# MathThyMod/GP_emu_UQSA

Hardware: AMD Instinct MI355X
Metric: log-marginal-likelihood evals/sec at n=16384 d=10 fp64; 1/2/4/8 GPU (higher is better)
Workload: dtype f64

## Files before the change

### gp_emu_uqsa_amd/csrc/gpemu.hip

```cpp
#include <hip/hip_runtime.h>

#include <algorithm>
#include <array>
#include <atomic>
#include <map>
#include <cmath>
#include <cstdio>
#include <cstdlib>
#include <cstring>
#include <limits>
#include <string>
#include <vector>

#include "../../include/gpemu.h"
#include "gpemu_kernels.hpp"
#include "gpemu_small.hpp"
#include "gpemu_tiny.hpp"
#include "gpemu_snb.hpp"
#include "gpemu_ozaki.hpp"
#include "gpemu_pivchol.hpp"
#include "gpemu_postgrad.hpp"
#include "gpemu_host_alloc.hpp"

using namespace gpe;
// ... 112 lines not shown
  size_t xs_cap = 0, xsw_cap = 0;
  double* dsmall = nullptr;
  double* dtiny = nullptr;
  int tiny_ek = 0, tiny_eg = 0;
  bool tiny_dirty = true;
  double* dsnb = nullptr;
  long long snb_np = 0;
  int snb_hc = 0, snb_mf = 0;
  bool snb_dirty = true;
  double onel_tag = 0.0;
  int oz_on = 1, oz_nmod = OZ_MAXMOD;
  int oz_min_np = 6144;
  int oz_np2 = 0, oz_list_len = 0;
  long long oz_npad = 0;
  OzConst oz_c{};
  int8_t* dozp = nullptr;
  int8_t* dozr = nullptr;
  int* dozx = nullptr;
  unsigned* dozl = nullptr;
  double* dozt = nullptr;
  hipEvent_t ev_oz = nullptr;
  std::vector<OzTriPair> oz_tri;
  int oz_tri_min = 8192;
  double oz_lauum_ops = 0.0;
  int oz_chol = 1, oz_chol_min = OZ_CHOL_MIN;
  OzTriPair oz_chol_q{};
  long long oz_chol_loff = 0;
  int oz_chol_llen = 0;
  double oz_chol_ops = 0.0;
  bool oz_chol_ready = false;
  bool oz_l21_valid = false;
  std::vector<hipEvent_t> oev;
  size_t oev_used = 0;
  double oz_ms = 0.0, oz_launches = 0.0, oz_ops = 0.0, oz_flops64 = 0.0;
  int dbg_skip_wait = -1;
  size_t small_cap = 0;

  double* hpin = nullptr;
  size_t hpin_cap = 0;

  float* dX32 = nullptr;
  size_t x32_cap = 0;
  bool x32_valid = false;
  float* dK32 = nullptr;
  size_t k32_cap = 0;
  hipEvent_t ev_pipe[2] = {nullptr, nullptr};
// ... 145 lines not shown
    return fail(c, GPE_ERR_ARG, "internal error: bad correlation family");
  if (a.d > 32) {
    const dim3 g(nblocks), b(256);
    if (a.fam == FAM_MATERN32) hipLaunchKernelGGL(k_pairs_wide<FAM_MATERN32>, g, b, 0, c->stream, a);
    else if (a.fam == FAM_MATERN52) hipLaunchKernelGGL(k_pairs_wide<FAM_MATERN52>, g, b, 0, c->stream, a);
    else hipLaunchKernelGGL(k_pairs_wide<FAM_GAUSS>, g, b, 0, c->stream, a);
    HIPCHK(c, hipGetLastError());
    return GPE_OK;
  }
  static constexpr int widths[] = {2, 4, 6, 8, 10, 12, 16, 20, 24, 32};
  int dm = 32;
  for (int w : widths)
    if (a.d <= w) { dm = w; break; }
  PairArgs a2 = a;
  while (a2.csplit < 4 && nblocks * a2.csplit * 2 <= 512) a2.csplit *= 2;
  const dim3 g(nblocks * a2.csplit), b(256);
  if (a.fam == FAM_MATERN32) launch_pairs_fam<FAM_MATERN32>(dm, g, b, c->stream, a2);
  else if (a.fam == FAM_MATERN52) launch_pairs_fam<FAM_MATERN52>(dm, g, b, c->stream, a2);
  else launch_pairs_fam<FAM_GAUSS>(dm, g, b, c->stream, a2);
  HIPCHK(c, hipGetLastError());
  return GPE_OK;
}

template <int FAM>
static void launch_contract(gpe_ctx* c, int d, int P, dim3 gc, int nblk, const double* rdiag, int cs) {
  const long long np = c->n_pad;
  const int bucket = std::max(d, P);
  if (d > 32 || P > 33) {
    hipLaunchKernelGGL(k_contract_wide<FAM>, dim3(nblk), dim3(256), 0, c->stream, c->tr.A, np, c->dXw, d, c->dWa, np, P, (int)c->n, c->dcpart, c->dinfo, 0, 0ll, rdiag);
  } else if (d == 10 && P <= 13) {
    hipLaunchKernelGGL((k_contract<10, 13, FAM>), gc, dim3(256), 0, c->stream, c->tr.A, np, c->dXw, d, c->dWa, np, P, (int)c->n, c->dcpart, c->dinfo, 0, 0ll, rdiag, cs);
  } else if (bucket <= 8) {
    hipLaunchKernelGGL((k_contract<8, 9, FAM>), gc, dim3(256), 0, c->stream, c->tr.A, np, c->dXw, d, c->dWa, np, P, (int)c->n, c->dcpart, c->dinfo, 0, 0ll, rdiag, cs);
  } else if (bucket <= 16) {
    hipLaunchKernelGGL((k_contract<16, 17, FAM>), gc, dim3(256), 0, c->stream, c->tr.A, np, c->dXw, d, c->dWa, np, P, (int)c->n, c->dcpart, c->dinfo, 0, 0ll, rdiag, cs);
  } else {
    hipLaunchKernelGGL((k_contract<32, 33, FAM>), gc, dim3(256), 0, c->stream, c->tr.A, np, c->dXw, d, c->dWa, np, P, (int)c->n, c->dcpart, c->dinfo, 0, 0ll, rdiag, cs);
  }
}

int launch_gemm_range(gpe_ctx* c, const Launch& L, hipStream_t st = nullptr) {
  if (!st) st = c->stream;
  const size_t lds = G_LDS_LAUNCH_DOUBLES * sizeof(double);
  const GemmProb* pr = c->dprobs + L.first;
  const unsigned* tl = (L.list >= 0) ? c->dtiles + L.list : nullptr;
  if (c->prof) {
    if (c->gev_used + 2 > c->gev.size()) {
      for (int i = 0; i < 256; ++i) {
        hipEvent_t e;
        HIPCHK(c, hipEventCreate(&e));
        c->gev.push_back(e);
      }
    }
    HIPCHK(c, hipEventRecord(c->gev[c->gev_used], st));
  }
  const dim3 g(L.tiles), b(256);
  if (L.cdef) {
    switch (L.kind) {
      case 0: hipLaunchKernelGGL((k_gemm<false, false, false, true>), g, b, lds, st, pr, L.count, tl, c->dinfo, L.ticket); break;
      case 1: hipLaunchKernelGGL((k_gemm<true, false, false, true>), g, b, lds, st, pr, L.count, tl, c->dinfo, L.ticket); break;
// ... 1131 lines not shown
    c->oz_chol_q = q;
    c->oz_chol_loff = (long long)all.size();
    c->oz_chol_llen = (int)ls.size();
    all.insert(all.end(), ls.begin(), ls.end());
    c->oz_chol_ops = 2.0 * OZ_T * OZ_T * (double)q.Pa * N * (nts * (nts + 1) / 2);
    planes = std::max(planes, (size_t)N * q.Pb * q.Pa);
    resid = std::max(resid, (size_t)N * (nts * (size_t)(nts + 1) / 2) * OZ_T * OZ_T);
    nex = std::max(nex, (size_t)q.Pb);
    c->oz_chol_ready = true;
  }
  CHK(dalloc(c, &c->dozp, planes));
  CHK(dalloc(c, &c->dozr, resid));
  CHK(dalloc(c, &c->dozx, nex));
  CHK(dalloc(c, &c->dozt, scratch));
  CHK(dalloc(c, &c->dozl, all.size()));
  HIPCHK(c, hipMemcpy(c->dozl, all.data(), all.size() * sizeof(unsigned), hipMemcpyHostToDevice));
  c->oz_c = oz_consts(N, np2);
  c->oz_np2 = np2;
  c->oz_npad = c->n_pad;
  return GPE_OK;
}

int oz_gemm_crt(gpe_ctx* c, const OzGemm& g, const OzCrt& r, int nti, double ops, double flops64,
                hipStream_t st = nullptr) {
  if (!st) st = c->stream;
  const OzConst& k = c->oz_c;
  if (c->prof) {
    while (c->oev_used + 2 > c->oev.size()) {
      hipEvent_t e;
      HIPCHK(c, hipEventCreate(&e));
      c->oev.push_back(e);
    }
    HIPCHK(c, hipEventRecord(c->oev[c->oev_used], st));
  }
  hipLaunchKernelGGL(k_oz_gemm, dim3(k.nmod * g.list_len), dim3(256), OZ_LDS, st, g, k);
  if (c->prof) {
    HIPCHK(c, hipEventRecord(c->oev[c->oev_used + 1], st));
    c->oev_used += 2;
    c->oz_launches += 1.0;
    c->oz_ops += ops;
    c->oz_flops64 += flops64;
  }
  hipLaunchKernelGGL(k_oz_crt, dim3((g.tri ? nti * (nti + 1) / 2 : nti * g.ntj) * 16), dim3(256), 0, st, r, k);
  HIPCHK(c, hipGetLastError());
  return GPE_OK;
}

int chol_schur(gpe_ctx* c, Fact& F, hipStream_t st, bool with_aug) {
  const Plan& pl = F.plan;
  const OzTriPair& q = c->oz_chol_q;
  if (!c->oz_chol_ready || q.h != pl.split_h) return fail(c, GPE_ERR_STATE, "internal error: split Cholesky without an int8 plan");
  if (with_aug) CHK(launch_gemm_range(c, pl.launches[pl.aug_mid], st));
  const long long ld = F.n_pad;
  oz_l21_launch(st, c->oz_c, q, F.A + (long long)q.h * TILE, ld, c->dozp, c->dozx);
  HIPCHK(c, hipGetLastError());
  const int nts = q.Pb / OZ_T;
  const long long pA = (long long)q.Pb * q.Pa, rb = (long long)nts * (nts + 1) / 2 * OZ_T * OZ_T;
  OzGemm g;
  g.a = g.b = OzOpnd{c->dozp, pA, q.Pa, 0};
  g.list = c->dozl + c->oz_chol_loff;
  g.list_len = c->oz_chol_llen;
  g.K = q.Pa;
  g.kbeg = 0;
  g.kend = 0;
  g.tri = 1;
  g.ntj = 0;
  g.res = c->dozr;
  g.res_bytes = rb;
  OzCrt r{c->dozr, rb, 1, 0, c->dozx, c->dozx, F.A + (long long)q.h * TILE * (ld + 1), ld, q.Rb, q.Rb, 1, -1.0};
  r.acc = 1;
  CHK(oz_gemm_crt(c, g, r, nts, c->oz_chol_ops, (double)q.Rb * q.Rb * q.Ra, st));
  c->oz_l21_valid = true;
  return GPE_OK;
}

int lauum_ozaki(gpe_ctx* c, Fact& F) {
  CHK(oz_prepare(c, F));
  const int np = (int)F.n_pad, np2 = c->oz_np2, NT2 = np2 / OZ_T;
  const OzConst& k = c->oz_c;
  const long long pb = oz_plane_bytes(np2), rb = (long long)NT2 * (NT2 + 1) / 2 * OZ_T * OZ_T;
  c->oz_l21_valid = false;
  hipLaunchKernelGGL(k_oz_colexp, dim3((np2 + 3) / 4), dim3(256), 0, c->stream, F.B, (long long)F.n_pad, np, np2,
                     k.beta, c->dozx);
  hipLaunchKernelGGL(k_oz_split, dim3(np2, (np2 + 256 * OZ_SPLIT_ROWS - 1) / (256 * OZ_SPLIT_ROWS)), dim3(256), 0,
                     c->stream, F.B, (long long)F.n_pad, np, np2, c->dozx, c->dozp, pb, k);
  OzGemm g;
  g.a = g.b = OzOpnd{c->dozp, pb, 0, np2};
  g.list = c->dozl;
  g.list_len = c->oz_list_len;
  g.K = np2;
  g.kbeg = 1;
  g.kend = 0;
  g.tri = 1;
  g.ntj = 0;
  g.res = c->dozr;
  g.res_bytes = rb;
  OzCrt r{c->dozr, rb, 1, 0, c->dozx, c->dozx, F.A, (long long)F.n_pad, np, np, 1, 1.0};
  return oz_gemm_crt(c, g, r, NT2, c->oz_lauum_ops, (double)np * np * np / 3.0);
}

const OzTriPair* oz_pair(const gpe_ctx* c, int t0, int h, int t1) {
  for (const OzTriPair& q : c->oz_tri)
    if (q.t0 == t0 && q.h == h && q.t1 == t1) return &q;
  return nullptr;
}

int oz_l21(gpe_ctx* c, Fact& F, const OzTriPair& q, hipStream_t st) {
  c->oz_l21_valid = false;
  oz_l21_launch(st, c->oz_c, q, F.A + (long long)q.h * TILE + (long long)q.t0 * TILE * F.n_pad, F.n_pad, c->dozp, c->dozx);
  HIPCHK(c, hipGetLastError());
  return GPE_OK;
}

int oz_l21_ahead(gpe_ctx* c, Fact& F, int t0, int h, int t1) {
  CHK(oz_prepare(c, F));
  const OzTriPair* q = oz_pair(c, t0, h, t1);
  if (!q) return fail(c, GPE_ERR_STATE, "internal error: TRTRI pair without an int8 plan");
  if (!c->ev_oz) HIPCHK(c, hipEventCreateWithFlags(&c->ev_oz, hipEventDisableTiming));
  HIPCHK(c, hipEventRecord(c->ev_fork, c->stream));
  HIPCHK(c, hipStreamWaitEvent(c->stream2, c->ev_fork, 0));
  CHK(oz_l21(c, F, *q, c->stream2));
// ... 88 lines not shown
  gpe_ctx* c = new gpe_ctx();
  c->device = device;
  c->aux.desc_base = AUX_DESC_BASE;
  {
    const char* ea = std::getenv("GPEMU_AUG");
    c->tr.aug = !(ea && std::string(ea) == "0");
  }
  {
    const char* e2 = std::getenv("GPEMU_POTRF");
    if (e2) {
      const std::string m(e2);
      c->potrf_group = m == "group" || m == "auto";
      c->potrf_mode = m == "group" ? 1 : (m == "auto" ? 0 : 2);
    }
    if (const char* eg = std::getenv("GPEMU_GROUP_P0")) c->grp_p0 = std::max(1, std::atoi(eg));
    if (const char* eg = std::getenv("GPEMU_GROUP_STRIDE")) c->grp_stride = std::max(0, std::atoi(eg));
    if (const char* ep = std::getenv("GPEMU_CHOL_PRIO")) c->chol_prio = std::atoi(ep) != 0;
    if (const char* et = std::getenv("GPEMU_TINY")) c->tiny = std::atoi(et) != 0;
    if (const char* ed = std::getenv("GPEMU_DEBUG_SKIP_WAIT")) c->dbg_skip_wait = std::atoi(ed);
    if (const char* eo = std::getenv("GPEMU_OZAKI")) c->oz_on = std::atoi(eo) != 0;
    if (const char* en = std::getenv("GPEMU_OZAKI_MIN_NP")) c->oz_min_np = std::max(512, std::atoi(en));
    if (const char* em = std::getenv("GPEMU_OZAKI_MODULI")) c->oz_nmod = std::max(8, std::min(OZ_MAXMOD, std::atoi(em)));
    if (const char* et = std::getenv("GPEMU_OZAKI_TRI_MIN")) c->oz_tri_min = std::max(512, std::atoi(et));
    if (const char* ec = std::getenv("GPEMU_OZAKI_CHOL")) c->oz_chol = std::max(0, std::min(3, std::atoi(ec)));
    if (const char* ec = std::getenv("GPEMU_OZAKI_CHOL_MIN")) c->oz_chol_min = std::max(256, std::atoi(ec));
    if (const char* es = std::getenv("GPEMU_POTRF_SB")) {
      c->potrf_sb = std::max(1, std::min(8, std::atoi(es)));
      if (const char* colon = std::strchr(es, ':')) c->potrf_sb_min = std::max(0, std::atoi(colon + 1));
    }
    if (const char* e3 = std::getenv("GPEMU_POTRF_W")) {
      c->potrf_groups.clear();
      std::string spec(e3);
      size_t pos = 0;
      while (pos < spec.size()) {
        size_t end = spec.find(',', pos);
        if (end == std::string::npos) end = spec.size();
        const std::string item = spec.substr(pos, end - pos);
        const size_t colon = item.find(':');
        const int w = std::atoi(item.substr(0, colon).c_str());
        const int lim = colon == std::string::npos ? 0 : std::atoi(item.substr(colon + 1).c_str());
        if (w >= 1 && w <= 8) c->potrf_groups.push_back({w, lim});
        pos = end + 1;
      }
    }
  }
  if (hipSetDevice(device) != hipSuccess || hipStreamCreateWithFlags(&c->stream, hipStreamNonBlocking) != hipSuccess ||
// ... 431 lines not shown
    c->gev_used = 0;
    c->gemm_launches = c->gemm_flops = c->gemm_ms = 0.0;
    c->oev_used = 0;
    c->oz_ms = c->oz_launches = c->oz_ops = c->oz_flops64 = 0.0;
  }
  const bool one_launch = c->tiny && kernel_fam(kernel) == FAM_GAUSS;
  if (one_launch && c->NB == 1 && d <= TINY_DM && q + 1 <= TINY_DM)
    return tiny_objective(c, gp4ml, kernel, hp, n_hp, fitnug, nu, s2, rscale, want_grad != 0, llh_out, grad_out,
                          sigma2_out);
  if (one_launch && c->NB >= 2 && c->NB <= SNB_MAXNB && d <= TINY_DM && q + 1 <= TINY_DM)
    return snb_objective(c, gp4ml, kernel, hp, n_hp, fitnug, nu, s2, rscale, want_grad != 0, llh_out, grad_out,
                         sigma2_out);

  CHK(factor_and_invert(c, kernel, hp, nu, s2, rscale, want_grad != 0, true));
  const int P = q + 1;
  const long long np = c->n_pad;
  const int NBt = c->tr.NB;
  CHK(ensure_pinned(c, (size_t)P * P + NBt + 64));
  CHK(gram_async(c, c->dZ, np, P, (int)np));
  HIPCHK(c, hipMemcpyAsync(c->hpin + P * P, c->tr.logdet, NBt * sizeof(double), hipMemcpyDeviceToHost, c->stream));
  HIPCHK(c, hipMemcpyAsync(c->hpin + P * P + NBt, c->dinfo, sizeof(int), hipMemcpyDeviceToHost, c->stream));
  HIPCHK(c, hipEventRecord(c->ev_host, c->stream));
  ev_rec(c, 4);
  if (want_grad) CHK(oz_use(c) ? lauum_ozaki(c, c->tr) : lauum(c, c->tr));
  ev_rec(c, 5);
  HIPCHK(c, hipEventSynchronize(c->ev_host));
  std::vector<double> G(c->hpin, c->hpin + (size_t)P * P);
  int info = 0;
  std::memcpy(&info, c->hpin + P * P + NBt, sizeof(int));
  if (info == GEMM_WAIT_TIMEOUT) return fail(c, GPE_ERR_HIP, "internal error: Cholesky panel wait timed out");
  double logdetA = 0.0;
  for (int k = 0; k < NBt; ++k) logdetA += c->hpin[P * P + k];
  logdetA *= 2.0;
  if (info != 0) {
    c->err = "matrix not positive definite (pivot " + std::to_string(info) + ")";
    return GPE_NOT_PD;
  }
  SmallAlgebra sa = small_from_gram(G, P);
  if (!sa.ok) {
    c->err = "H^T A^-1 H not positive definite";
    return GPE_NOT_PD;
  }
  const double n = (double)c->n;
  double llh, sig2, cfac, gscale;
  if (gp4ml) {
    llh = 0.5 * (sa.quad + logdetA + sa.logdetQ + (n - q) * std::log(2.0 * M_PI));
    sig2 = s2;
// ... 7 lines not shown
  }
  *llh_out = llh;
  if (sigma2_out) *sigma2_out = sig2;
  if (!want_grad) {
    ev_rec(c, 6);
    ev_rec(c, 7);
    goto done;
  }
  {
    CHK(ensure_pinned(c, (size_t)P * P + 8));
    const std::vector<double> T2 = small_t2(sa, q, cfac);
    std::memcpy(c->hpin, T2.data(), T2.size() * sizeof(double));
    HIPCHK(c, hipMemcpyAsync(c->dT2, c->hpin, T2.size() * sizeof(double), hipMemcpyHostToDevice, c->stream));
    CHK(apply_small(c, c->dZ, np, P, c->dT2, P, c->dR2, np, (int)np, c->dinfo));
    CHK(skinny(c, true, c->tr.B, np, c->NB, c->NB, true, c->dR2, np, P, c->dWa, np));
    ev_rec(c, 6);
    const double* rdiag = (gp4ml && !kernel_alt(kernel) && c->has_r) ? c->dr : nullptr;
    const int nblk = c->NB * (c->NB + 1) / 2;
    int cs = 1;
    if (!(d > 32 || P > 33))
      while (cs < 4 && nblk * cs * 2 <= 512) cs *= 2;
    const dim3 gc(nblk * cs);
    const int fam = kernel_fam(kernel);
    if (fam == FAM_MATERN32) launch_contract<FAM_MATERN32>(c, d, P, gc, nblk, rdiag, cs);
    else if (fam == FAM_MATERN52) launch_contract<FAM_MATERN52>(c, d, P, gc, nblk, rdiag, cs);
    else launch_contract<FAM_GAUSS>(c, d, P, gc, nblk, rdiag, cs);
    HIPCHK(c, hipGetLastError());
    hipLaunchKernelGGL(k_reduce_rows, dim3(d + 3), dim3(256), 0, c->stream, c->dcpart, nblk * cs, d + 3, c->dcsum);
    HIPCHK(c, hipGetLastError());
    ev_rec(c, 7);
    HIPCHK(c, hipMemcpyAsync(c->hpin, c->dcsum, (d + 3) * sizeof(double), hipMemcpyDeviceToHost, c->stream));
    HIPCHK(c, hipStreamSynchronize(c->stream));
    const double* red = c->hpin;
    double coff, cdiag;
    kernel_consts(kernel, nu, true, &coff, &cdiag);
    small_grad(red, d, kernel_alt(kernel), nu, fitnug, gp4ml, gscale, s2, coff, cdiag, n_hp,
               grad_out, rdiag != nullptr);
  }
done:
  if (c->prof) {
    HIPCHK(c, hipStreamSynchronize(c->stream));
    float ms;
    const int pairs[7][2] = {{0, 1}, {1, 2}, {2, 3}, {4, 5}, {3, 4}, {5, 7}, {0, 7}};
    for (int i = 0; i < 7; ++i) {
      ms = 0.f;
      (void)hipEventElapsedTime(&ms, c->ev[pairs[i][0]], c->ev[pairs[i][1]]);
      c->phase_ms[i] = ms;
    }
    double g = 0.0;
// ... 80 lines not shown
    c->pl_len = (int)l.size();
    c->pl_nti = nti;
    c->pl_ntj = ntj;
  }
  CHK(grow_buf(c, &c->dpkp, &c->pkp_cap, (size_t)N * pB));
  CHK(grow_buf(c, &c->dpke, &c->pke_cap, (size_t)mp2));
  CHK(grow_buf(c, &c->dpres, &c->pres_cap, (size_t)N * rb));
  hipLaunchKernelGGL(k_oz_rowexp<false>, dim3(mp2 / 4), dim3(256), 0, st, Ks, (long long)np, (int)mp, mp2, np, 0, k.beta,
                     c->dpke);
  hipLaunchKernelGGL(k_oz_split_rect<false>, dim3(mp2, (np2 + 2047) / 2048), dim3(256), 0, st, Ks, (long long)np,
                     (int)mp, np, 0, c->dpke, c->dpkp, pB, (long long)np2, np2, k);
  OzGemm g;
  g.a = OzOpnd{c->dpxp, (long long)np2 * np2, np2, 0};
  g.b = OzOpnd{c->dpkp, pB, np2, 0};
  g.list = c->dpl;
  g.list_len = c->pl_len;
  g.K = np2;
  g.kbeg = 0;
  g.kend = 1;
  g.tri = 0;
  g.ntj = ntj;
  g.res = c->dpres;
  g.res_bytes = rb;
  hipLaunchKernelGGL(k_oz_gemm, dim3(N * g.list_len), dim3(256), OZ_LDS, st, g, k);
  OzCrt r{c->dpres, rb, 0, ntj, c->dpxe, c->dpke, V, (long long)np, np, (int)mp, 0, 1.0};
  hipLaunchKernelGGL(k_oz_crt, dim3((unsigned)(nti * ntj * 16)), dim3(256), 0, st, r, k);
  HIPCHK(c, hipGetLastError());
  return GPE_OK;
}

static int ensure_ainv(gpe_ctx* c) {
  if (c->ainv_valid) return GPE_OK;
  CHK(ensure_linv(c));
  CHK(lauum(c, c->tr));
  c->ainv_valid = true;
  return GPE_OK;
}

int gpe_solve(gpe_ctx* c, int32_t ncols, const double* B, double* X) {
  CHK(check_ready(c));
  if (!c->factor_valid) return fail(c, GPE_ERR_STATE, "no resident factor (call gpe_factor)");
  if (ncols <= 0 || !B || !X) return fail(c, GPE_ERR_ARG, "bad solve args");
  CHK(ensure_linv(c));
  const long long np = c->n_pad, n = c->n;
  for (int c0 = 0; c0 < ncols; c0 += SK_PMAX) {
    const int cc = std::min(SK_PMAX, ncols - c0);
// ... 1197 lines not shown
```

### gp_emu_uqsa_amd/csrc/gpemu_ozaki.hpp

```cpp
#pragma once
#include <algorithm>
#include <array>
#include <cmath>
#include <cstdlib>
#include <cstring>
#include <utility>
#include <vector>

namespace gpe {

constexpr int OZ_T = 256;
constexpr int OZ_SK = 64;
constexpr int OZ_NBUF = 4;
constexpr int OZ_OPND = OZ_T * OZ_SK;
constexpr int OZ_LDS = OZ_NBUF * 2 * OZ_OPND;
constexpr int OZ_MAXMOD = 16;
constexpr int OZ_MAX_K = (1 << 17) - 128;

struct OzConst {
  int m[OZ_MAXMOD];
  int c16[OZ_MAXMOD];
  float inv[OZ_MAXMOD];
  double rhi[OZ_MAXMOD];
  double rlo[OZ_MAXMOD];
  double Md;
  int nmod;
// ... 79 lines not shown
  long long ld;
  int np2;
};
__device__ __forceinline__ const int8_t* oz_tile_rows(const OzOpnd& o, int t, int k, long long& ld) {
  if (o.ld == 0) {
    ld = o.np2 - OZ_T * t;
    return o.p + oz_panel_off(t, o.np2) + (k - OZ_T * t);
  }
  ld = o.ld;
  return o.p + (long long)OZ_T * t * o.ld + k;
}

struct OzGemm {
  OzOpnd a, b;
  const unsigned* list;
  int list_len;
  int K, kbeg, kend;
  int tri, ntj;
  int8_t* res;
  long long res_bytes;
  int kdiv = 1;
  int ti0 = 0;
};
__device__ __forceinline__ long long oz_res_tile(int tri, int ntj, int ti, int tj) {
  return tri ? (long long)ti * (ti + 1) / 2 + tj : (long long)ti * ntj + tj;
}

static __global__ void __launch_bounds__(256, 1) k_oz_gemm(OzGemm g, OzConst cst) {
  extern __shared__ __attribute__((aligned(16))) double lds_d[];
  int8_t* lds = reinterpret_cast<int8_t*>(lds_d);
  const int l = (int)blockIdx.x / g.list_len;
  const unsigned ent = g.list[(int)blockIdx.x - l * g.list_len];
  if (ent == 0xffffffffu) return;
  const int ti = (int)(ent >> 16), tj = (int)(ent & 0xffffu);
  const int kb = g.kbeg == 1 ? OZ_T * ti : (g.kbeg == 2 ? OZ_T * tj : (g.kbeg == 3 ? 128 * ((2 * ti) / g.kdiv) : 0));
  const int ke = g.kend == 1 ? min(g.K, OZ_T * (ti + 1)) : g.K;
  const int tid = threadIdx.x, lane = tid & 63;
  const int wave = __builtin_amdgcn_readfirstlane(tid >> 6);
  const int wm = (wave >> 1) * 128, wn = (wave & 1) * 128;
  OzOpnd oa = g.a, ob = g.b;
  oa.p += (long long)l * oa.plane_bytes;
  ob.p += (long long)l * ob.plane_bytes;
  long long lda, ldb;
  const int kp = (lane & 3) ^ ((lane >> 4) & 3);
  const int8_t* sa = oz_tile_rows(oa, ti, kb, lda);
  const int8_t* sb = oz_tile_rows(ob, tj, kb, ldb);
  sa += (long long)(16 * wave + (lane >> 2)) * lda + 16 * kp;
  sb += (long long)(16 * wave + (lane >> 2)) * ldb + 16 * kp;
  auto stage = [&](int s) {
    int8_t* As = lds + (s & (OZ_NBUF - 1)) * 2 * OZ_OPND;
    int8_t* Bs = As + OZ_OPND;
#pragma unroll
    for (int p = 0; p < 4; ++p) {
      const int w = wave + 4 * p;
      oz_glds16(sa + (long long)p * 64 * lda + (long long)s * OZ_SK, As + 16 * w * OZ_SK);
      oz_glds16(sb + (long long)p * 64 * ldb + (long long)s * OZ_SK, Bs + 16 * w * OZ_SK);
    }
  };
  oz_v16i acc[4][4];
// ... 117 lines not shown
    const double rh = cst.rhi[l], rl = cst.rlo[l];
#pragma unroll
    for (int r = 0; r < 16; ++r) {
      const double cv = (double)(int)(int8_t)((unsigned)w[r >> 2] >> (8 * (r & 3)));
      shi[r] = fma(cv, rh, shi[r]);
      slo[r] = fma(cv, rl, slo[r]);
    }
  }
  const int em = g.exr[gm];
  const double sc = g.alpha * cst.Md;
#pragma unroll
  for (int r = 0; r < 16; ++r) {
    const int gn = gn0 + (r & 3) + 8 * (r >> 2);
    if (gn >= g.cols || (g.lower128 && (gm >> 7) < (gn >> 7))) continue;
    const double v = (shi[r] - rint(shi[r])) + slo[r];
    const int en = g.exc[gn];
    double* dst = g.C + (gm - OZ_T * g.ti0 + (long long)gn * g.ldc);
    const double s = ldexp(sc, -(em + en));
    if (em == OZ_EX_NAN || en == OZ_EX_NAN) *dst = __builtin_nan("");
    else *dst = g.acc ? fma(v, s, *dst) : v * s;
  }
}

__device__ __forceinline__ bool oz_keep(int mask, int r, int k) {
  return mask == 1 ? k >= r : (mask == 2 ? k <= r : true);
}

template <bool TRANS>
static __global__ void __launch_bounds__(256) k_oz_rowexp(const double* __restrict__ src, long long ld, int R, int Rp,
                                                          int Kv, int mask, int beta, int* __restrict__ ex) {
  if constexpr (!TRANS) {
    const int lane = threadIdx.x & 63, r = blockIdx.x * 4 + (threadIdx.x >> 6);
    if (r >= Rp) return;
    double mx = 0.0;
    if (r < R)
      for (int k = lane; k < Kv; k += 64)
        if (oz_keep(mask, r, k)) mx = oz_pmax(mx, fabs(src[k + (long long)r * ld]));
    for (int off = 32; off > 0; off >>= 1) mx = oz_pmax(mx, __shfl_xor(mx, off, 64));
    if (lane == 0) ex[r] = oz_ex_of(mx, beta);
  } else {
    __shared__ double red[4][64];
    const int rl = threadIdx.x & 63, q = threadIdx.x >> 6, r = blockIdx.x * 64 + rl;
    const int k0 = blockIdx.y * 256;
    double mx = 0.0;
    if (r < R)
#pragma unroll 8
      for (int u = 0; u < 64; ++u) {
        const int k = k0 + 4 * u + q;
        if (k < Kv && oz_keep(mask, r, k)) mx = oz_pmax(mx, fabs(src[r + (long long)k * ld]));
      }
    red[q][rl] = mx;
    __syncthreads();
    if (q == 0 && r < R) {
      mx = oz_pmax(oz_pmax(red[0][rl], red[1][rl]), oz_pmax(red[2][rl], red[3][rl]));
      if (!(mx <= 1.7976931348623157e308)) atomicMax(ex + r, OZ_IL_BAD);
      else if (mx > 0.0) atomicMax(ex + r, ilogb(mx) + 2048);
    }
  }
}
static __global__ void __launch_bounds__(256) k_oz_il_to_ex(int* __restrict__ ex, int Rp, int beta) {
  const int r = blockIdx.x * 256 + threadIdx.x;
  if (r < Rp) ex[r] = ex[r] >= OZ_IL_BAD ? OZ_EX_NAN : (ex[r] > 0 ? (beta - 1) - (ex[r] - 2048) : 0);
}

__device__ __forceinline__ unsigned oz_res8(double x, double m, double im, int mi) {
  const double q = rint(x * im);
  int r = (int)fma(-q, m, x);
  r = r > 127 ? r - mi : (r < -128 ? r + mi : r);
  return (unsigned)r & 0xffu;
}

template <bool TRANS>
static __global__ void __launch_bounds__(256) k_oz_split_rect(const double* __restrict__ src, long long ld, int R,
                                                              int Kv, int mask, const int* __restrict__ ex,
                                                              int8_t* __restrict__ planes, long long plane_bytes,
                                                              long long ldp, int Kp, OzConst cst) {
  if constexpr (!TRANS) {
    const int r = blockIdx.x;
    const int k0 = ((int)blockIdx.y * 256 + (int)threadIdx.x) * 8;
    if (k0 >= Kp) return;
    const int e = ex[r];
    double xs[8];
    const double* p = src + k0 + (long long)r * ld;
    const int side = mask == 1 ? (k0 >= r ? 1 : (k0 + 7 < r ? 0 : 2))
                   : (mask == 2 ? (k0 + 7 <= r ? 1 : (k0 > r ? 0 : 2)) : 1);
    if (r < R && k0 + 8 <= Kv && side == 1 && ((reinterpret_cast<uintptr_t>(p) & 15) == 0)) {
#pragma unroll
      for (int u = 0; u < 8; u += 2) {
        const double2 v = *reinterpret_cast<const double2*>(p + u);
        xs[u] = v.x;
        xs[u + 1] = v.y;
      }
    } else {
#pragma unroll
      for (int u = 0; u < 8; ++u) {
        const int k = k0 + u;
        xs[u] = (side != 0 && r < R && k < Kv && oz_keep(mask, r, k)) ? p[u] : 0.0;
      }
    }
#pragma unroll
    for (int u = 0; u < 8; ++u) xs[u] = e == OZ_EX_NAN ? 0.0 : rint(ldexp(xs[u], e));
    int8_t* dst = planes + (long long)r * ldp + k0;
    for (int l = 0; l < cst.nmod; ++l) {
      const double m = (double)cst.m[l], im = 1.0 / m;
      unsigned w0 = 0u, w1 = 0u;
#pragma unroll
      for (int u = 0; u < 4; ++u) {
        w0 |= oz_res8(xs[u], m, im, cst.m[l]) << (8 * u);
        w1 |= oz_res8(xs[u + 4], m, im, cst.m[l]) << (8 * u);
      }
      *reinterpret_cast<uint2*>(dst + (long long)l * plane_bytes) = make_uint2(w0, w1);
    }
  } else {
    __shared__ __attribute__((aligned(16))) unsigned tr[64 * 20];
    const int lane = threadIdx.x & 63, rp = lane & 31, kg = (int)threadIdx.x >> 5;
    const int r = (int)blockIdx.x * 64 + 2 * rp;
    const int k0 = (int)blockIdx.y * 64 + 8 * kg;
    const int e0 = ex[r], e1 = ex[r + 1];
    double x0[8], x1[8];
    const double* p = src + r + (long long)k0 * ld;
    const bool vec = r + 1 < R && ((reinterpret_cast<uintptr_t>(src + r) & 15) == 0) && (ld & 1) == 0;
#pragma unroll
    for (int u = 0; u < 8; ++u) {
      const int k = k0 + u;
      double a = 0.0, b = 0.0;
      if (k < Kv) {
        if (vec) {
          const double2 v = *reinterpret_cast<const double2*>(p + (long long)u * ld);
          a = v.x;
          b = v.y;
        } else {
          if (r < R) a = p[(long long)u * ld];
          if (r + 1 < R) b = p[(long long)u * ld + 1];
        }
      }
      x0[u] = oz_keep(mask, r, k) ? a : 0.0;
      x1[u] = oz_keep(mask, r + 1, k) ? b : 0.0;
    }
#pragma unroll
    for (int u = 0; u < 8; ++u) {
// ... 79 lines not shown
  std::vector<std::vector<unsigned>> bins(8);
  std::vector<double> load(8, 0.0);
  for (const Blk& b : blks) {
    const int x = (int)(std::min_element(load.begin(), load.end()) - load.begin());
    load[x] += b.w;
    bins[x].insert(bins[x].end(), b.t.begin(), b.t.end());
  }
  size_t longest = 0;
  for (auto& b : bins) longest = std::max(longest, b.size());
  std::vector<unsigned> list(8 * longest, 0xffffffffu);
  for (int x = 0; x < 8; ++x)
    for (size_t q = 0; q < bins[x].size(); ++q) list[8 * q + x] = bins[x][q];
  return list;
}

inline std::vector<std::array<int, 3>> trtri_level_pairs(int NB, int s) {
  std::vector<std::array<int, 3>> prs;
  for (int t0 = 0; t0 < NB; t0 += s) {
    const int h = t0 + s / 2;
    if (h >= NB) continue;
    prs.push_back({t0, h, std::min(t0 + s, NB)});
  }
  return prs;
}

struct OzTriPair {
  int t0, h, t1, Ra, Rb, Pa, Pb;
  long long la_off, lb_off;
  int la_len, lb_len;
  double ops_a, ops_b;
  size_t planes_bytes(int N) const { return (size_t)N * Pa * (Pa + Pb); }
  size_t resid_bytes(int N) const { return (size_t)N * Pa * Pb; }
};
inline OzTriPair oz_tri_pair_plan(int t0, int h, int t1, int N, std::vector<unsigned>& lists) {
  OzTriPair q;
  q.t0 = t0; q.h = h; q.t1 = t1;
  q.Ra = (h - t0) * TILE;
  q.Rb = (t1 - h) * TILE;
  q.Pa = (q.Ra + OZ_T - 1) / OZ_T * OZ_T;
  q.Pb = (q.Rb + OZ_T - 1) / OZ_T * OZ_T;
  const int nti = q.Pb / OZ_T, ntj = q.Pa / OZ_T;
  const std::vector<unsigned> la = oz_list(nti, ntj, false, [&](int, int tj) { return (double)(q.Pa - OZ_T * tj); });
  const std::vector<unsigned> lb = oz_list(nti, ntj, false, [&](int ti, int) { return (double)(OZ_T * (ti + 1)); });
  q.ops_a = q.ops_b = 0.0;
  for (int tj = 0; tj < ntj; ++tj) q.ops_a += 2.0 * OZ_T * OZ_T * nti * (double)(q.Pa - OZ_T * tj) * N;
  for (int ti = 0; ti < nti; ++ti) q.ops_b += 2.0 * OZ_T * OZ_T * ntj * (double)(OZ_T * (ti + 1)) * N;
// ... 9 lines not shown
inline void oz_l21_launch(hipStream_t st, const OzConst& k, const OzTriPair& q, const double* L21, long long ld,
                          int8_t* planes, int* ex) {
  const long long pA = (long long)q.Pb * q.Pa;
  (void)hipMemsetAsync(ex, 0, q.Pb * sizeof(int), st);
  hipLaunchKernelGGL(k_oz_rowexp<true>, dim3(q.Pb / 64, (q.Ra + 255) / 256), dim3(256), 0, st, L21, ld, q.Rb, q.Pb,
                     q.Ra, 0, k.beta, ex);
  hipLaunchKernelGGL(k_oz_il_to_ex, dim3((q.Pb + 255) / 256), dim3(256), 0, st, ex, q.Pb, k.beta);
  hipLaunchKernelGGL(k_oz_split_rect<true>, dim3(q.Pb / 64, q.Pa / 64), dim3(256), 0, st, L21, ld, q.Rb, q.Ra, 0,
                     ex, planes, pA, (long long)q.Pa, q.Pa, k);
}

template <class GC>
void oz_tri_pair_launches(hipStream_t st, const OzConst& k, const OzTriPair& q, const unsigned* lists, const double* L21,
                          const double* X11, const double* X22, double* X21, long long ld, double* T, int8_t* planes,
                          int8_t* res, int* ex, bool l21_done, GC gc) {
  int* exA = ex;
  int* exB = ex + q.Pb;
  const int nti = q.Pb / OZ_T, ntj = q.Pa / OZ_T;
  const long long rb = (long long)nti * ntj * OZ_T * OZ_T;
  {
    const long long pA = (long long)q.Pb * q.Pa, pB = (long long)q.Pa * q.Pa;
    int8_t* PA = planes;
    int8_t* PB = planes + (size_t)k.nmod * pA;
    if (!l21_done) oz_l21_launch(st, k, q, L21, ld, PA, exA);
    hipLaunchKernelGGL(k_oz_rowexp<false>, dim3(q.Pa / 4), dim3(256), 0, st, X11, ld, q.Ra, q.Pa, q.Ra, 1, k.beta, exB);
    hipLaunchKernelGGL(k_oz_split_rect<false>, dim3(q.Pa, (q.Pa + 2047) / 2048), dim3(256), 0, st, X11, ld, q.Ra, q.Ra,
                       1, exB, PB, pB, (long long)q.Pa, q.Pa, k);
    OzGemm g;
    g.a = OzOpnd{PA, pA, q.Pa, 0};
    g.b = OzOpnd{PB, pB, q.Pa, 0};
    g.list = lists + q.la_off;
    g.list_len = q.la_len;
    g.K = q.Pa;
    g.kbeg = 2;
    g.kend = 0;
    g.tri = 0;
    g.ntj = ntj;
    g.res = res;
    g.res_bytes = rb;
    OzCrt r{res, rb, 0, ntj, exA, exB, T, (long long)q.Pb, q.Rb, q.Ra, 0, 1.0};
    gc(g, r, nti, q.ops_a, (double)q.Ra * q.Ra * q.Rb);
  }
  {
    const long long pA = (long long)q.Pb * q.Pb, pB = (long long)q.Pa * q.Pb;
    int8_t* PA = planes;
    int8_t* PB = planes + (size_t)k.nmod * pA;
    (void)hipMemsetAsync(exA, 0, q.Pb * sizeof(int), st);
    hipLaunchKernelGGL(k_oz_rowexp<true>, dim3(q.Pb / 64, (q.Rb + 255) / 256), dim3(256), 0, st, X22, ld, q.Rb, q.Pb,
                       q.Rb, 2, k.beta, exA);
    hipLaunchKernelGGL(k_oz_il_to_ex, dim3((q.Pb + 255) / 256), dim3(256), 0, st, exA, q.Pb, k.beta);
    hipLaunchKernelGGL(k_oz_rowexp<false>, dim3(q.Pa / 4), dim3(256), 0, st, T, (long long)q.Pb, q.Ra, q.Pa, q.Rb, 0,
                       k.beta, exB);
    hipLaunchKernelGGL(k_oz_split_rect<true>, dim3(q.Pb / 64, q.Pb / 64), dim3(256), 0, st, X22, ld, q.Rb, q.Rb, 2,
                       exA, PA, pA, (long long)q.Pb, q.Pb, k);
    hipLaunchKernelGGL(k_oz_split_rect<false>, dim3(q.Pa, (q.Pb + 2047) / 2048), dim3(256), 0, st, T, (long long)q.Pb,
                       q.Ra, q.Rb, 0, exB, PB, pB, (long long)q.Pb, q.Pb, k);
    OzGemm g;
    g.a = OzOpnd{PA, pA, q.Pb, 0};
    g.b = OzOpnd{PB, pB, q.Pb, 0};
    g.list = lists + q.lb_off;
    g.list_len = q.lb_len;
    g.K = q.Pb;
    g.kbeg = 0;
    g.kend = 1;
    g.tri = 0;
    g.ntj = ntj;
    g.res = res;
    g.res_bytes = rb;
    OzCrt r{res, rb, 0, ntj, exA, exB, X21, ld, q.Rb, q.Ra, 0, -1.0};
    gc(g, r, nti, q.ops_b, (double)q.Rb * q.Rb * q.Ra);
  }
}

}
```

Measured before the change: 17.52.

## Fuse Ozaki LAUUM CRT reconstruction into gradient contraction kernel; skip masked plane work

Adds a k_oz_contract kernel that rebuilds the inverse entries straight from the int8 modular residues and exponents while computing the gradient contraction. This makes the separate k_oz_crt pass and the write and re-read of the fp64 LAUUM result unnecessary when the Ozaki path is active. The triangular-masked rowexp and split kernels also exit early for tiles the mask never reads. A host-side check aborts if masked planes are handed to a product whose k-range does not match. The fused kernel does heavier per-element reconstruction math inside the contraction, which may add register pressure.

```diff
diff --git a/gp_emu_uqsa_amd/csrc/gpemu.hip b/gp_emu_uqsa_amd/csrc/gpemu.hip
--- a/gp_emu_uqsa_amd/csrc/gpemu.hip
+++ b/gp_emu_uqsa_amd/csrc/gpemu.hip
@@ -158,6 +158,7 @@
   hipEvent_t ev_oz = nullptr;
   std::vector<OzTriPair> oz_tri;
   int oz_tri_min = 8192;
+  int oz_fuse = 1;
   double oz_lauum_ops = 0.0;
   int oz_chol = 1, oz_chol_min = OZ_CHOL_MIN;
   OzTriPair oz_chol_q{};
@@ -349,20 +350,33 @@
   return GPE_OK;
 }
 
+template <int DMAX, int QMAX, int FAM>
+static void launch_contract_bucket(gpe_ctx* c, int d, int P, dim3 gc, const double* rdiag, int cs, bool oz) {
+  const long long np = c->n_pad;
+  if (oz) {
+    const int NT2 = c->oz_np2 / OZ_T;
+    hipLaunchKernelGGL((k_oz_contract<DMAX, QMAX, FAM>), gc, dim3(256), 0, c->stream, c->dozr,
+                       (long long)NT2 * (NT2 + 1) / 2 * OZ_T * OZ_T, c->dozx, c->oz_c, c->dXw, d, c->dWa, np, P, (int)c->n,
+                       c->dcpart, c->dinfo, rdiag, cs);
+  } else {
+    hipLaunchKernelGGL((k_contract<DMAX, QMAX, FAM>), gc, dim3(256), 0, c->stream, c->tr.A, np, c->dXw, d, c->dWa, np, P, (int)c->n, c->dcpart, c->dinfo, 0, 0ll, rdiag, cs);
+  }
+}
+
 template <int FAM>
-static void launch_contract(gpe_ctx* c, int d, int P, dim3 gc, int nblk, const double* rdiag, int cs) {
+static void launch_contract(gpe_ctx* c, int d, int P, dim3 gc, int nblk, const double* rdiag, int cs, bool oz) {
   const long long np = c->n_pad;
   const int bucket = std::max(d, P);
   if (d > 32 || P > 33) {
     hipLaunchKernelGGL(k_contract_wide<FAM>, dim3(nblk), dim3(256), 0, c->stream, c->tr.A, np, c->dXw, d, c->dWa, np, P, (int)c->n, c->dcpart, c->dinfo, 0, 0ll, rdiag);
   } else if (d == 10 && P <= 13) {
-    hipLaunchKernelGGL((k_contract<10, 13, FAM>), gc, dim3(256), 0, c->stream, c->tr.A, np, c->dXw, d, c->dWa, np, P, (int)c->n, c->dcpart, c->dinfo, 0, 0ll, rdiag, cs);
+    launch_contract_bucket<10, 13, FAM>(c, d, P, gc, rdiag, cs, oz);
   } else if (bucket <= 8) {
-    hipLaunchKernelGGL((k_contract<8, 9, FAM>), gc, dim3(256), 0, c->stream, c->tr.A, np, c->dXw, d, c->dWa, np, P, (int)c->n, c->dcpart, c->dinfo, 0, 0ll, rdiag, cs);
+    launch_contract_bucket<8, 9, FAM>(c, d, P, gc, rdiag, cs, oz);
   } else if (bucket <= 16) {
-    hipLaunchKernelGGL((k_contract<16, 17, FAM>), gc, dim3(256), 0, c->stream, c->tr.A, np, c->dXw, d, c->dWa, np, P, (int)c->n, c->dcpart, c->dinfo, 0, 0ll, rdiag, cs);
+    launch_contract_bucket<16, 17, FAM>(c, d, P, gc, rdiag, cs, oz);
   } else {
-    hipLaunchKernelGGL((k_contract<32, 33, FAM>), gc, dim3(256), 0, c->stream, c->tr.A, np, c->dXw, d, c->dWa, np, P, (int)c->n, c->dcpart, c->dinfo, 0, 0ll, rdiag, cs);
+    launch_contract_bucket<32, 33, FAM>(c, d, P, gc, rdiag, cs, oz);
   }
 }
 
@@ -1540,7 +1554,7 @@
 }
 
 int oz_gemm_crt(gpe_ctx* c, const OzGemm& g, const OzCrt& r, int nti, double ops, double flops64,
-                hipStream_t st = nullptr) {
+                hipStream_t st = nullptr, bool crt = true) {
   if (!st) st = c->stream;
   const OzConst& k = c->oz_c;
   if (c->prof) {
@@ -1559,7 +1573,7 @@
     c->oz_ops += ops;
     c->oz_flops64 += flops64;
   }
-  hipLaunchKernelGGL(k_oz_crt, dim3((g.tri ? nti * (nti + 1) / 2 : nti * g.ntj) * 16), dim3(256), 0, st, r, k);
+  if (crt) hipLaunchKernelGGL(k_oz_crt, dim3((g.tri ? nti * (nti + 1) / 2 : nti * g.ntj) * 16), dim3(256), 0, st, r, k);
   HIPCHK(c, hipGetLastError());
   return GPE_OK;
 }
@@ -1592,7 +1606,7 @@
   return GPE_OK;
 }
 
-int lauum_ozaki(gpe_ctx* c, Fact& F) {
+int lauum_ozaki(gpe_ctx* c, Fact& F, bool crt = true) {
   CHK(oz_prepare(c, F));
   const int np = (int)F.n_pad, np2 = c->oz_np2, NT2 = np2 / OZ_T;
   const OzConst& k = c->oz_c;
@@ -1614,7 +1628,7 @@
   g.res = c->dozr;
   g.res_bytes = rb;
   OzCrt r{c->dozr, rb, 1, 0, c->dozx, c->dozx, F.A, (long long)F.n_pad, np, np, 1, 1.0};
-  return oz_gemm_crt(c, g, r, NT2, c->oz_lauum_ops, (double)np * np * np / 3.0);
+  return oz_gemm_crt(c, g, r, NT2, c->oz_lauum_ops, (double)np * np * np / 3.0, nullptr, crt);
 }
 
 const OzTriPair* oz_pair(const gpe_ctx* c, int t0, int h, int t1) {
@@ -1749,6 +1763,7 @@
     if (const char* en = std::getenv("GPEMU_OZAKI_MIN_NP")) c->oz_min_np = std::max(512, std::atoi(en));
     if (const char* em = std::getenv("GPEMU_OZAKI_MODULI")) c->oz_nmod = std::max(8, std::min(OZ_MAXMOD, std::atoi(em)));
     if (const char* et = std::getenv("GPEMU_OZAKI_TRI_MIN")) c->oz_tri_min = std::max(512, std::atoi(et));
+    if (const char* ef = std::getenv("GPEMU_OZ_FUSE_CONTRACT")) c->oz_fuse = std::atoi(ef) != 0;
     if (const char* ec = std::getenv("GPEMU_OZAKI_CHOL")) c->oz_chol = std::max(0, std::min(3, std::atoi(ec)));
     if (const char* ec = std::getenv("GPEMU_OZAKI_CHOL_MIN")) c->oz_chol_min = std::max(256, std::atoi(ec));
     if (const char* es = std::getenv("GPEMU_POTRF_SB")) {
@@ -2226,7 +2241,8 @@
   HIPCHK(c, hipMemcpyAsync(c->hpin + P * P + NBt, c->dinfo, sizeof(int), hipMemcpyDeviceToHost, c->stream));
   HIPCHK(c, hipEventRecord(c->ev_host, c->stream));
   ev_rec(c, 4);
-  if (want_grad) CHK(oz_use(c) ? lauum_ozaki(c, c->tr) : lauum(c, c->tr));
+  const bool fuse = oz_use(c) && c->oz_fuse && d <= 32 && P <= 33;
+  if (want_grad) CHK(oz_use(c) ? lauum_ozaki(c, c->tr, !fuse) : lauum(c, c->tr));
   ev_rec(c, 5);
   HIPCHK(c, hipEventSynchronize(c->ev_host));
   std::vector<double> G(c->hpin, c->hpin + (size_t)P * P);
@@ -2280,9 +2296,9 @@
       while (cs < 4 && nblk * cs * 2 <= 512) cs *= 2;
     const dim3 gc(nblk * cs);
     const int fam = kernel_fam(kernel);
-    if (fam == FAM_MATERN32) launch_contract<FAM_MATERN32>(c, d, P, gc, nblk, rdiag, cs);
-    else if (fam == FAM_MATERN52) launch_contract<FAM_MATERN52>(c, d, P, gc, nblk, rdiag, cs);
-    else launch_contract<FAM_GAUSS>(c, d, P, gc, nblk, rdiag, cs);
+    if (fam == FAM_MATERN32) launch_contract<FAM_MATERN32>(c, d, P, gc, nblk, rdiag, cs, fuse);
+    else if (fam == FAM_MATERN52) launch_contract<FAM_MATERN52>(c, d, P, gc, nblk, rdiag, cs, fuse);
+    else launch_contract<FAM_GAUSS>(c, d, P, gc, nblk, rdiag, cs, fuse);
     HIPCHK(c, hipGetLastError());
     hipLaunchKernelGGL(k_reduce_rows, dim3(d + 3), dim3(256), 0, c->stream, c->dcpart, nblk * cs, d + 3, c->dcsum);
     HIPCHK(c, hipGetLastError());
@@ -2409,6 +2425,7 @@
   g.ntj = ntj;
   g.res = c->dpres;
   g.res_bytes = rb;
+  oz_mask_matches(2, c->dpxp, g);
   hipLaunchKernelGGL(k_oz_gemm, dim3(N * g.list_len), dim3(256), OZ_LDS, st, g, k);
   OzCrt r{c->dpres, rb, 0, ntj, c->dpxe, c->dpke, V, (long long)np, np, (int)mp, 0, 1.0};
   hipLaunchKernelGGL(k_oz_crt, dim3((unsigned)(nti * ntj * 16)), dim3(256), 0, st, r, k);
diff --git a/gp_emu_uqsa_amd/csrc/gpemu_ozaki.hpp b/gp_emu_uqsa_amd/csrc/gpemu_ozaki.hpp
--- a/gp_emu_uqsa_amd/csrc/gpemu_ozaki.hpp
+++ b/gp_emu_uqsa_amd/csrc/gpemu_ozaki.hpp
@@ -2,6 +2,7 @@
 #include <algorithm>
 #include <array>
 #include <cmath>
+#include <cstdio>
 #include <cstdlib>
 #include <cstring>
 #include <utility>
@@ -127,6 +128,10 @@
   int kdiv = 1;
   int ti0 = 0;
 };
+__host__ __device__ __forceinline__ void oz_k_range(int kbeg, int kend, int kdiv, int K, int ti, int tj, int& kb, int& ke) {
+  kb = kbeg == 1 ? OZ_T * ti : (kbeg == 2 ? OZ_T * tj : (kbeg == 3 ? 128 * ((2 * ti) / kdiv) : 0));
+  ke = kend == 1 ? (K < OZ_T * (ti + 1) ? K : OZ_T * (ti + 1)) : K;
+}
 __device__ __forceinline__ long long oz_res_tile(int tri, int ntj, int ti, int tj) {
   return tri ? (long long)ti * (ti + 1) / 2 + tj : (long long)ti * ntj + tj;
 }
@@ -138,8 +143,8 @@
   const unsigned ent = g.list[(int)blockIdx.x - l * g.list_len];
   if (ent == 0xffffffffu) return;
   const int ti = (int)(ent >> 16), tj = (int)(ent & 0xffffu);
-  const int kb = g.kbeg == 1 ? OZ_T * ti : (g.kbeg == 2 ? OZ_T * tj : (g.kbeg == 3 ? 128 * ((2 * ti) / g.kdiv) : 0));
-  const int ke = g.kend == 1 ? min(g.K, OZ_T * (ti + 1)) : g.K;
+  int kb, ke;
+  oz_k_range(g.kbeg, g.kend, g.kdiv, g.K, ti, tj, kb, ke);
   const int tid = threadIdx.x, lane = tid & 63;
   const int wave = __builtin_amdgcn_readfirstlane(tid >> 6);
   const int wm = (wave >> 1) * 128, wn = (wave & 1) * 128;
@@ -303,9 +308,134 @@
   }
 }
 
+template <int DMAX, int QMAX, int FAM>
+static __global__ void __launch_bounds__(256) k_oz_contract(const int8_t* __restrict__ res, long long res_bytes,
+                                                            const int* __restrict__ ex, OzConst cst,
+                                                            const double* xw, int d, const double* Wa, long long ldw,
+                                                            int q1, int n_valid, double* part, const int* abort_flag,
+                                                            const double* rdiag, int csplit) {
+  __shared__ double xs[TILE * DMAX];
+  __shared__ double ws[TILE * QMAX];
+  __shared__ double red[4 * (DMAX + 3)];
+  __shared__ int exs[TILE];
+  if (abort_flag && *abort_flag) return;
+  int ti, tj;
+  const int share = (int)blockIdx.x % csplit;
+  const int blk = (int)blockIdx.x / csplit;
+  tri_decode(blk, ti, tj);
+  const int tid = threadIdx.x;
+  for (int e = tid; e < TILE * DMAX; e += 256) {
+    const int c = e / DMAX, k = e - c * DMAX;
+    xs[e] = k < d ? xw[(long long)(tj * TILE + c) * d + k] : 0.0;
+  }
+  for (int e = tid; e < TILE * QMAX; e += 256) {
+    const int c = e / QMAX, k = e - c * QMAX;
+    ws[e] = k < q1 ? Wa[(long long)(tj * TILE + c) + (long long)k * ldw] : 0.0;
+  }
+  if (tid < TILE) exs[tid] = ex[tj * TILE + tid];
+  const int lane = tid & 63, wave = tid >> 6;
+  const int r = 32 * wave + (lane & 31);
+  const int gi = ti * TILE + r;
+  double xi[DMAX], wi[QMAX], acc[DMAX];
+#pragma unroll
+  for (int k = 0; k < DMAX; ++k) {
+    xi[k] = (k < d) ? xw[(long long)gi * d + k] : 0.0;
+    acc[k] = 0.0;
+  }
+#pragma unroll
+  for (int k = 0; k < QMAX; ++k) wi[k] = (k < q1) ? Wa[gi + (long long)k * ldw] : 0.0;
+  double accE = 0.0, accT = 0.0, accR = 0.0;
+  const double ri = (rdiag && gi < n_valid && ti == tj) ? rdiag[gi] : 0.0;
+  __syncthreads();
+  if (gi < n_valid) {
+    const int Ti = ti >> 1, Tj = tj >> 1, sub = 2 * (ti & 1) + (tj & 1);
+    const int8_t* src = res + ((long long)Ti * (Ti + 1) / 2 + Tj) * (OZ_T * OZ_T) +
+                        ((long long)(16 * sub + 4 * wave) * 64 + lane) * 16;
+    const int em = ex[gi];
+    const int cw = TILE / csplit, cbeg = share * cw;
+    const int cend = min(min((ti == tj) ? r + 1 : TILE, n_valid - tj * TILE), cbeg + cw);
+    for (int j = cbeg / 32; j < (cbeg + cw) / 32; ++j) {
+      const int cj = 32 * j + 4 * (lane >> 5);
+      if (cj >= cend) continue;
+      double shi[16], slo[16];
+#pragma unroll
+      for (int u = 0; u < 16; ++u) shi[u] = slo[u] = 0.0;
+#pragma unroll 4
+      for (int l = 0; l < cst.nmod; ++l) {
+        const oz_v4i w = *reinterpret_cast<const oz_v4i*>(src + (long long)j * (64 * 16) + (long long)l * res_bytes);
+        const double rh = cst.rhi[l], rl = cst.rlo[l];
+#pragma unroll
+        for (int u = 0; u < 16; ++u) {
+          const double cv = (double)(int)(int8_t)((unsigned)w[u >> 2] >> (8 * (u & 3)));
+          shi[u] = fma(cv, rh, shi[u]);
+          slo[u] = fma(cv, rl, slo[u]);
+        }
+      }
+#pragma unroll
+      for (int u = 0; u < 16; ++u) {
+        const int c = cj + (u & 3) + 8 * (u >> 2);
+        if (c >= cend) continue;
+        const int gj = tj * TILE + c;
+        const double v = (shi[u] - rint(shi[u])) + slo[u];
+        const int en = exs[c];
+        double mij = __dmul_rn(v, ldexp(cst.Md, -(em + en)));
+        if (em == OZ_EX_NAN || en == OZ_EX_NAN) mij = __builtin_nan("");
+#pragma unroll
+        for (int k = 0; k < QMAX; ++k) mij = fma(-wi[k], ws[c * QMAX + k], mij);
+        double df2[DMAX];
+        double s = 0.0;
+#pragma unroll
+        for (int k = 0; k < DMAX; ++k) {
+          const double df = xi[k] - xs[c * DMAX + k];
+          df2[k] = df * df;
+          s += df2[k];
+        }
+        const bool dg = gj == gi;
+        accT += dg ? mij : 0.0;
+        accR += dg ? mij * ri : 0.0;
+        if constexpr (FAM == FAM_GAUSS) {
+          const double me = dg ? 0.0 : mij * exp(-s);
+          accE += me;
+#pragma unroll
+          for (int k = 0; k < DMAX; ++k) acc[k] = fma(me, df2[k], acc[k]);
+        } else {
+          double rho, g;
+          matern_rho_g<FAM>(s, rho, g);
+          accE += dg ? 0.0 : mij * rho;
+          const double mg = dg ? 0.0 : mij * g;
+#pragma unroll
+          for (int k = 0; k < DMAX; ++k) acc[k] = fma(mg, df2[k], acc[k]);
+        }
+      }
+    }
+  }
+  const int nv = d + 3;
+  for (int k = 0; k < nv; ++k) {
+    double v = 0.0;
+#pragma unroll
+    for (int kk = 0; kk < DMAX; ++kk)
+      if (kk == k) v = acc[kk];
+    if (k == d) v = accE;
+    if (k == d + 1) v = accT;
+    if (k == d + 2) v = accR;
+    for (int off = 32; off > 0; off >>= 1) v += __shfl_down(v, off, 64);
+    if (lane == 0) red[wave * (DMAX + 3) + k] = v;
+  }
+  __syncthreads();
+  if (tid < nv) {
+    const double s = (red[tid] + red[(DMAX + 3) + tid]) + (red[2 * (DMAX + 3) + tid] + red[3 * (DMAX + 3) + tid]);
+    part[((long long)blk * csplit + share) * nv + tid] = s;
+  }
+}
+
 __device__ __forceinline__ bool oz_keep(int mask, int r, int k) {
   return mask == 1 ? k >= r : (mask == 2 ? k <= r : true);
 }
+__host__ __device__ __forceinline__ bool oz_plane_read(int mask, int r, int k) {
+  return mask == 1 ? k >= OZ_T * (r / OZ_T) : (mask == 2 ? k < OZ_T * (r / OZ_T + 1) : true);
+}
+__host__ __device__ __forceinline__ bool oz_rect_thread_writes(int mask, int r, int k0) { return oz_plane_read(mask, r, k0 + 7); }
+__host__ __device__ __forceinline__ bool oz_rect_block_writes(int mask, int r0, int k0) { return oz_plane_read(mask, r0, k0); }
 
 template <bool TRANS>
 static __global__ void __launch_bounds__(256) k_oz_rowexp(const double* __restrict__ src, long long ld, int R, int Rp,
@@ -315,7 +445,7 @@
     if (r >= Rp) return;
     double mx = 0.0;
     if (r < R)
-      for (int k = lane; k < Kv; k += 64)
+      for (int k = (mask == 1 ? (r & ~63) : 0) + lane; k < (mask == 2 ? min(Kv, r + 1) : Kv); k += 64)
         if (oz_keep(mask, r, k)) mx = oz_pmax(mx, fabs(src[k + (long long)r * ld]));
     for (int off = 32; off > 0; off >>= 1) mx = oz_pmax(mx, __shfl_xor(mx, off, 64));
     if (lane == 0) ex[r] = oz_ex_of(mx, beta);
@@ -323,6 +453,7 @@
     __shared__ double red[4][64];
     const int rl = threadIdx.x & 63, q = threadIdx.x >> 6, r = blockIdx.x * 64 + rl;
     const int k0 = blockIdx.y * 256;
+    if ((mask == 2 && k0 > (int)blockIdx.x * 64 + 63) || (mask == 1 && k0 + 255 < (int)blockIdx.x * 64)) return;
     double mx = 0.0;
     if (r < R)
 #pragma unroll 8
@@ -359,7 +490,7 @@
   if constexpr (!TRANS) {
     const int r = blockIdx.x;
     const int k0 = ((int)blockIdx.y * 256 + (int)threadIdx.x) * 8;
-    if (k0 >= Kp) return;
+    if (k0 >= Kp || !oz_rect_thread_writes(mask, r, k0)) return;
     const int e = ex[r];
     double xs[8];
     const double* p = src + k0 + (long long)r * ld;
@@ -397,6 +528,7 @@
     const int lane = threadIdx.x & 63, rp = lane & 31, kg = (int)threadIdx.x >> 5;
     const int r = (int)blockIdx.x * 64 + 2 * rp;
     const int k0 = (int)blockIdx.y * 64 + 8 * kg;
+    if (!oz_rect_block_writes(mask, (int)blockIdx.x * 64, (int)blockIdx.y * 64)) return;
     const int e0 = ex[r], e1 = ex[r + 1];
     double x0[8], x1[8];
     const double* p = src + r + (long long)k0 * ld;
@@ -522,6 +654,16 @@
     prs.push_back({t0, h, std::min(t0 + s, NB)});
   }
   return prs;
+}
+
+inline void oz_mask_matches(int mask, const int8_t* planes, const OzGemm& g) {
+  const bool ok = mask == 1 ? (g.kbeg == 2 && g.kend == 0 && g.b.p == planes)
+                            : (mask == 2 ? (g.kbeg == 0 && g.kend == 1 && g.a.p == planes) : true);
+  if (!ok) {
+    std::fprintf(stderr, "gpemu: masked int8 planes (mask %d) given to a product with kbeg %d, kend %d\n", mask, g.kbeg,
+                 g.kend);
+    std::abort();
+  }
 }
 
 struct OzTriPair {
@@ -577,10 +719,6 @@
     const long long pA = (long long)q.Pb * q.Pa, pB = (long long)q.Pa * q.Pa;
     int8_t* PA = planes;
     int8_t* PB = planes + (size_t)k.nmod * pA;
-    if (!l21_done) oz_l21_launch(st, k, q, L21, ld, PA, exA);
-    hipLaunchKernelGGL(k_oz_rowexp<false>, dim3(q.Pa / 4), dim3(256), 0, st, X11, ld, q.Ra, q.Pa, q.Ra, 1, k.beta, exB);
-    hipLaunchKernelGGL(k_oz_split_rect<false>, dim3(q.Pa, (q.Pa + 2047) / 2048), dim3(256), 0, st, X11, ld, q.Ra, q.Ra,
-                       1, exB, PB, pB, (long long)q.Pa, q.Pa, k);
     OzGemm g;
     g.a = OzOpnd{PA, pA, q.Pa, 0};
     g.b = OzOpnd{PB, pB, q.Pa, 0};
@@ -593,6 +731,11 @@
     g.ntj = ntj;
     g.res = res;
     g.res_bytes = rb;
+    oz_mask_matches(1, PB, g);
+    if (!l21_done) oz_l21_launch(st, k, q, L21, ld, PA, exA);
+    hipLaunchKernelGGL(k_oz_rowexp<false>, dim3(q.Pa / 4), dim3(256), 0, st, X11, ld, q.Ra, q.Pa, q.Ra, 1, k.beta, exB);
+    hipLaunchKernelGGL(k_oz_split_rect<false>, dim3(q.Pa, (q.Pa + 2047) / 2048), dim3(256), 0, st, X11, ld, q.Ra, q.Ra,
+                       1, exB, PB, pB, (long long)q.Pa, q.Pa, k);
     OzCrt r{res, rb, 0, ntj, exA, exB, T, (long long)q.Pb, q.Rb, q.Ra, 0, 1.0};
     gc(g, r, nti, q.ops_a, (double)q.Ra * q.Ra * q.Rb);
   }
@@ -600,16 +743,6 @@
     const long long pA = (long long)q.Pb * q.Pb, pB = (long long)q.Pa * q.Pb;
     int8_t* PA = planes;
     int8_t* PB = planes + (size_t)k.nmod * pA;
-    (void)hipMemsetAsync(exA, 0, q.Pb * sizeof(int), st);
-    hipLaunchKernelGGL(k_oz_rowexp<true>, dim3(q.Pb / 64, (q.Rb + 255) / 256), dim3(256), 0, st, X22, ld, q.Rb, q.Pb,
-                       q.Rb, 2, k.beta, exA);
-    hipLaunchKernelGGL(k_oz_il_to_ex, dim3((q.Pb + 255) / 256), dim3(256), 0, st, exA, q.Pb, k.beta);
-    hipLaunchKernelGGL(k_oz_rowexp<false>, dim3(q.Pa / 4), dim3(256), 0, st, T, (long long)q.Pb, q.Ra, q.Pa, q.Rb, 0,
-                       k.beta, exB);
-    hipLaunchKernelGGL(k_oz_split_rect<true>, dim3(q.Pb / 64, q.Pb / 64), dim3(256), 0, st, X22, ld, q.Rb, q.Rb, 2,
-                       exA, PA, pA, (long long)q.Pb, q.Pb, k);
-    hipLaunchKernelGGL(k_oz_split_rect<false>, dim3(q.Pa, (q.Pb + 2047) / 2048), dim3(256), 0, st, T, (long long)q.Pb,
-                       q.Ra, q.Rb, 0, exB, PB, pB, (long long)q.Pb, q.Pb, k);
     OzGemm g;
     g.a = OzOpnd{PA, pA, q.Pb, 0};
     g.b = OzOpnd{PB, pB, q.Pb, 0};
@@ -622,6 +755,17 @@
     g.ntj = ntj;
     g.res = res;
     g.res_bytes = rb;
+    oz_mask_matches(2, PA, g);
+    (void)hipMemsetAsync(exA, 0, q.Pb * sizeof(int), st);
+    hipLaunchKernelGGL(k_oz_rowexp<true>, dim3(q.Pb / 64, (q.Rb + 255) / 256), dim3(256), 0, st, X22, ld, q.Rb, q.Pb,
+                       q.Rb, 2, k.beta, exA);
+    hipLaunchKernelGGL(k_oz_il_to_ex, dim3((q.Pb + 255) / 256), dim3(256), 0, st, exA, q.Pb, k.beta);
+    hipLaunchKernelGGL(k_oz_rowexp<false>, dim3(q.Pa / 4), dim3(256), 0, st, T, (long long)q.Pb, q.Ra, q.Pa, q.Rb, 0,
+                       k.beta, exB);
+    hipLaunchKernelGGL(k_oz_split_rect<true>, dim3(q.Pb / 64, q.Pb / 64), dim3(256), 0, st, X22, ld, q.Rb, q.Rb, 2,
+                       exA, PA, pA, (long long)q.Pb, q.Pb, k);
+    hipLaunchKernelGGL(k_oz_split_rect<false>, dim3(q.Pa, (q.Pb + 2047) / 2048), dim3(256), 0, st, T, (long long)q.Pb,
+                       q.Ra, q.Rb, 0, exB, PB, pB, (long long)q.Pb, q.Pb, k);
     OzCrt r{res, rb, 0, ntj, exA, exB, X21, ld, q.Rb, q.Ra, 0, -1.0};
     gc(g, r, nti, q.ops_b, (double)q.Rb * q.Rb * q.Ra);
   }
```

New measurement: 17.66, median of 6. No clear change (+0.8%).
